# bioinformatics-ua/polus

Measured on AMD Instinct MI355X. Metric: train samples/sec BioBERT-base NER seq256, higher is better.
Workload: dtype bf16; 1 GPU; BERT-base (L=12,H=768,A=12,I=3072,V=28996) token classification C=4, seq_len=256, 64 samples/GPU, AdamW lr 5e-5 wd 0.01 warm-up 10%, dropout 0.1 (hidden + attention) (BASELINE.json configs[2] per-GPU shape), random-init weights; global_batch=64, seq_len=256, parallelism=dp1, grad_allreduce=none

## Files before the change

polus_amd/csrc/common.h:

```cpp
#pragma once
#include <hip/hip_runtime.h>
#include <stdint.h>
#include <stdio.h>
#include <string.h>
#include <math.h>

#include "../../include/polus_hip.h"

typedef __bf16 bf16_t;
typedef __bf16 bf16x8 __attribute__((ext_vector_type(8)));
typedef __bf16 bf16x4 __attribute__((ext_vector_type(4)));
typedef short s16x4 __attribute__((ext_vector_type(4)));
typedef float f32x4 __attribute__((ext_vector_type(4)));

void polus_set_error(const char* fmt, ...);
#define POLUS_FAIL(...) do { polus_set_error(__VA_ARGS__); return POLUS_ERR_INVALID; } while (0)
#define POLUS_REQUIRE(cond, ...) do { if (!(cond)) { polus_set_error(__VA_ARGS__); return POLUS_ERR_INVALID; } } while (0)
#define POLUS_CHECK_LAUNCH(name) do { hipError_t e__ = hipGetLastError(); \
    if (e__ != hipSuccess) { polus_set_error("%s: launch failed: %s", name, hipGetErrorString(e__)); return POLUS_ERR_HIP; } } while (0)
#define POLUS_HIP(call) do { hipError_t e__ = (call); \
    if (e__ != hipSuccess) { polus_set_error("%s failed: %s", #call, hipGetErrorString(e__)); return POLUS_ERR_HIP; } } while (0)

static inline size_t polus_dtype_size(int dt) { return dt == POLUS_BF16 ? 2 : 4; }
static inline bool polus_aligned16(const void* p) { return (((uintptr_t)p) & 15) == 0; }

struct PolusCfg {
    int gemm_pp;
    int gemm_v1;
    int dw_ungrouped;
    int dw_fused_reduce;
    int ln_bwd_blocks;
    int ln_fin_single;
    int gemm_ring128;
    int gemm_auto_split;
    int ln_halfwave;
    int gemm_order;
    int gemm_persist;
    int reserve_cus;
    int attn_bwd_kres;
    int attn_debug;
    int dw_streamk;
    int dw_sk_cus;
    int dw_sk_delta;
    int attn_fused;
};
const PolusCfg& polus_cfg();
int polus_num_cus();
int polus_reserved_cus();

struct PolusDyn { uint32_t salt; float lr, lr_t; uint32_t pad; };
const PolusDyn* polus_dyn();
__device__ __forceinline__ uint32_t polus_eff_seed(uint32_t seed, const PolusDyn* dyn) {
    if (!dyn) return seed;
    uint32_t x = seed + dyn->salt;
    x ^= x >> 15;
    return x * 0x2C1B3C6Du;
}

template <typename T> __device__ __forceinline__ float to_f(T x);
template <> __device__ __forceinline__ float to_f<float>(float x) { return x; }
template <> __device__ __forceinline__ float to_f<bf16_t>(bf16_t x) { return (float)x; }
template <typename T> __device__ __forceinline__ T from_f(float x);
template <> __device__ __forceinline__ float from_f<float>(float x) { return x; }
template <> __device__ __forceinline__ bf16_t from_f<bf16_t>(float x) { return (bf16_t)x; }

template <typename T> __device__ __forceinline__ void load4(const T* p, float (&v)[4]);
template <> __device__ __forceinline__ void load4<float>(const float* p, float (&v)[4]) {
    float4 t = *reinterpret_cast<const float4*>(p); v[0] = t.x; v[1] = t.y; v[2] = t.z; v[3] = t.w;
}
template <> __device__ __forceinline__ void load4<bf16_t>(const bf16_t* p, float (&v)[4]) {
    bf16x4 t = *reinterpret_cast<const bf16x4*>(p);
    v[0] = (float)t[0]; v[1] = (float)t[1]; v[2] = (float)t[2]; v[3] = (float)t[3];
}
template <typename T> __device__ __forceinline__ void store4(T* p, const float (&v)[4]);
template <> __device__ __forceinline__ void store4<float>(float* p, const float (&v)[4]) {
    *reinterpret_cast<float4*>(p) = make_float4(v[0], v[1], v[2], v[3]);
}
template <> __device__ __forceinline__ void store4<bf16_t>(bf16_t* p, const float (&v)[4]) {
    bf16x4 t; t[0] = (bf16_t)v[0]; t[1] = (bf16_t)v[1]; t[2] = (bf16_t)v[2]; t[3] = (bf16_t)v[3];
    *reinterpret_cast<bf16x4*>(p) = t;
}

__device__ __forceinline__ float erf_fast(float x) {
    const float ax = fabsf(x);
    const float t = __frcp_rn(1.0f + 0.3275911f * ax);
    float poly = 1.061405429f;
    poly = poly * t - 1.453152027f;
    poly = poly * t + 1.421413741f;
    poly = poly * t - 0.284496736f;
    poly = poly * t + 0.254829592f;
    const float r = 1.0f - poly * t * __expf(-ax * ax);
    return copysignf(r, x);
}
__device__ __forceinline__ float gelu_f(float x) { return 0.5f * x * (1.0f + erf_fast(x * 0.70710678118654752f)); }
__device__ __forceinline__ float gelu_grad_f(float x) {
    float cdf = 0.5f * (1.0f + erf_fast(x * 0.70710678118654752f));
    float pdf = 0.3989422804014327f * __expf(-0.5f * x * x);
    return cdf + x * pdf;
}
__device__ __forceinline__ float swish_f(float x) { return x / (1.0f + __expf(-x)); }
__device__ __forceinline__ float swish_grad_f(float x) {
    float s = 1.0f / (1.0f + __expf(-x));
    return s * (1.0f + x * (1.0f - s));
}
typedef float f32x2_t __attribute__((ext_vector_type(2)));
__device__ __forceinline__ f32x2_t gelu_poly2(f32x2_t x, const float (&c)[11]) {
    f32x2_t xc = {__builtin_amdgcn_fmed3f(x[0], -4.5f, 4.5f), __builtin_amdgcn_fmed3f(x[1], -4.5f, 4.5f)};
    f32x2_t s = xc * xc;
    f32x2_t u = __builtin_elementwise_fma(s, (f32x2_t){2.0f / 20.25f, 2.0f / 20.25f}, (f32x2_t){-1.0f, -1.0f});
    f32x2_t r = {c[10], c[10]};
#pragma unroll
    for (int k = 9; k >= 0; --k) r = __builtin_elementwise_fma(r, u, (f32x2_t){c[k], c[k]});
    return __builtin_elementwise_fma(xc, r, (f32x2_t){0.5f, 0.5f});
}
__device__ __forceinline__ f32x2_t gelu_cdf2(f32x2_t x) {
    const float q[11] = {1.569049305e-01f, -7.719386095e-02f, 5.470119065e-02f, -4.010921159e-02f, 2.828393083e-02f,
                         -1.902094059e-02f, 1.143922652e-02f, -5.251548121e-03f, 2.716277400e-03f, -2.340015935e-03f,
                         9.806926012e-04f};
    return gelu_poly2(x, q);
}
__device__ __forceinline__ f32x2_t gelu_grad2(f32x2_t x) {
    const float w[11] = {1.594289755e-01f, -9.003904569e-02f, 8.714168751e-02f, -9.350841452e-02f, 9.645831298e-02f,
                         -9.557466143e-02f, 7.437658385e-02f, -3.356380937e-02f, 2.252388123e-02f, -3.068672777e-02f,
                         1.457471506e-02f};
    return gelu_poly2(x, w);
}
// ... 131 lines not shown
```

polus_amd/csrc/norm.hip:

```cpp
#include "common.h"

namespace {

constexpr int MAXC = 8;
constexpr int WAVES = 16;
constexpr int LN_THREADS = 64 * WAVES;
constexpr int MAX_PARTIAL_BLOCKS = 256;

__device__ __forceinline__ int n_chunks(int H) { return (H + 255) >> 8; }

template <typename T, int NC>
__device__ __forceinline__ void load_row(const T* row, int H, int lane, float (&v)[NC][4]) {
#pragma unroll
    for (int c = 0; c < NC; ++c) {
        int col = (lane + 64 * c) * 4;
        if (col < H) load4<T>(row + col, v[c]);
        else { v[c][0] = v[c][1] = v[c][2] = v[c][3] = 0.f; }
    }
}

template <int NC>
__device__ __forceinline__ void load_feat(const float* __restrict__ p, int H, int lane, float (&v)[NC][4]) {
#pragma unroll
    for (int c = 0; c < NC; ++c) {
// ... 170 lines not shown
    }
}

template <typename T, typename TDX, int NC>
__device__ __forceinline__ void ln_bwd_row(const float (&xv)[NC][4], const T* dyrow, const float (&gv)[NC][4],
                                           TDX* dxrow, int H, int lane, float mu, float rs, ColAcc<NC>& acc,
                                           int want_bias, TDX* dxm_row = nullptr, DropArgs out_drop = DropArgs{0, 0, 1.f},
                                           DropArgs in_drop = DropArgs{0, 0, 1.f}, unsigned rowbase = 0) {
    float dy[NC][4];
    load_row<T, NC>(dyrow, H, lane, dy);
    if (in_drop.thresh) {
#pragma unroll
        for (int c = 0; c < NC; ++c) {
            int col = (lane + 64 * c) * 4;
            polus_dropout_run<4>(dy[c], in_drop.seed, rowbase + col, in_drop.thresh, in_drop.inv, true);
        }
    }
    float s1 = 0.f, s2 = 0.f;
    float xh[NC][4], dxh[NC][4];
#pragma unroll
    for (int c = 0; c < NC; ++c) {
        int col = (lane + 64 * c) * 4;
        if (col < H) {
#pragma unroll
            for (int e = 0; e < 4; ++e) {
                xh[c][e] = (xv[c][e] - mu) * rs;
                dxh[c][e] = dy[c][e] * gv[c][e];
                s1 += dxh[c][e];
                s2 += dxh[c][e] * xh[c][e];
                acc.dg[c][e] += dy[c][e] * xh[c][e];
                acc.db[c][e] += dy[c][e];
            }
        } else {
#pragma unroll
            for (int e = 0; e < 4; ++e) xh[c][e] = dxh[c][e] = 0.f;
        }
    }
    s1 = wave_sum(s1) / (float)H;
    s2 = wave_sum(s2) / (float)H;
#pragma unroll
    for (int c = 0; c < NC; ++c) {
        int col = (lane + 64 * c) * 4;
        if (col < H) {
            float o[4], om[4];
#pragma unroll
            for (int e = 0; e < 4; ++e) { o[e] = (dxh[c][e] - s1 - xh[c][e] * s2) * rs; om[e] = o[e]; }
            if (out_drop.thresh) polus_dropout_run<4>(om, out_drop.seed, rowbase + col, out_drop.thresh, out_drop.inv, true);
            if (want_bias) {
#pragma unroll
                for (int e = 0; e < 4; ++e) acc.dbias[c][e] += om[e];
            }
            store4<TDX>(dxrow + col, o);
            if (dxm_row) store4<TDX>(dxm_row + col, om);
        }
    }
}

constexpr int BWD_WAVES = 4, BWD_MAX_BLOCKS = 1024, FIN_GROUP = 128;
template <typename T, int NC>
__global__ __launch_bounds__(64 * BWD_WAVES) void ln_bwd_kernel(const T* __restrict__ dy, const T* __restrict__ x,
                                                     const float* __restrict__ gamma, const float* __restrict__ mean,
                                                     const float* __restrict__ rstd, T* __restrict__ dx,
                                                     float* __restrict__ partial, int rows, int H, int want_bias,
                                                     T* __restrict__ dxm, DropArgs drop) {
    if (drop.thresh) drop.seed = polus_eff_seed(drop.seed, drop.dyn);
    extern __shared__ __attribute__((aligned(16))) unsigned char smem_raw[];
    float* lds = reinterpret_cast<float*>(smem_raw);
    const int lane = threadIdx.x & 63, wid = threadIdx.x >> 6;
    ColAcc<NC> acc;
    colacc_zero(acc);
    float gv[NC][4];
    load_feat<NC>(gamma, H, lane, gv);
    for (int row = blockIdx.x * BWD_WAVES + wid; row < rows; row += gridDim.x * BWD_WAVES) {
        float xv[NC][4];
        load_row<T, NC>(x + (long)row * H, H, lane, xv);
        ln_bwd_row<T, T, NC>(xv, dy + (long)row * H, gv, dx + (long)row * H, H, lane, mean[row], rstd[row], acc, want_bias,
                             dxm ? dxm + (long)row * H : nullptr, drop, DropArgs{0, 0, 1.f}, (unsigned)row * (unsigned)H);
    }
    colacc_flush_par<NC, BWD_WAVES>(acc, lds, partial, H, lane, wid, want_bias);
}

__global__ __launch_bounds__(1024) void colsum_finalize_kernel(const float* __restrict__ partial, int P, int pstride,
                                                               int ncols, int seg, float* out0, float* out1,
                                                               float* out2, int accumulate, int pgroup = 0) {
    __shared__ float red[16][64];
    const int cx = threadIdx.x & 63, gy = threadIdx.x >> 6;
    const int col = blockIdx.x * 64 + cx;
    float s = 0.f;
    if (pgroup > 0) {
        const int p0 = blockIdx.y * pgroup;
        partial += (long)p0 * pstride;
        P = min(pgroup, P - p0);
        out0 += (long)blockIdx.y * ncols;
    }
    if (col < ncols) {
#pragma unroll 8
        for (int p = gy; p < P; p += 16) s += partial[(long)p * pstride + col];
    }
    red[gy][cx] = s;
    __syncthreads();
    if (gy == 0 && col < ncols) {
        float t = 0.f;
#pragma unroll
        for (int k = 0; k < 16; ++k) t += red[k][cx];
        int which = col / seg, c = col % seg;
        float* out = which == 0 ? out0 : which == 1 ? out1 : out2;
        if (out) out[c] = accumulate ? out[c] + t : t;
    }
}

template <int NC>
__global__ __launch_bounds__(64 * BWD_WAVES) void ln_bwd_hw_kernel(const bf16_t* __restrict__ dy, const bf16_t* __restrict__ x,
                                                                    const float* __restrict__ gamma, const float* __restrict__ mean,
                                                                    const float* __restrict__ rstd, bf16_t* __restrict__ dx,
                                                                    float* __restrict__ partial, int rows, int H, int want_bias,
                                                                    bf16_t* __restrict__ dxm, DropArgs drop) {
    if (drop.thresh) drop.seed = polus_eff_seed(drop.seed, drop.dyn);
    extern __shared__ __attribute__((aligned(16))) unsigned char smem_raw[];
    float* lds = reinterpret_cast<float*>(smem_raw);
    const int lane = threadIdx.x & 63, wid = threadIdx.x >> 6, half = lane >> 5, hl = lane & 31;
    float gv[NC][8], adg[NC][8], adb[NC][8], abias[NC][8];
#pragma unroll
    for (int c = 0; c < NC; ++c) {
        const int col = (hl + 32 * c) * 8;
        load4<float>(gamma + col, *reinterpret_cast<float(*)[4]>(&gv[c][0])); load4<float>(gamma + col + 4, *reinterpret_cast<float(*)[4]>(&gv[c][4]));
#pragma unroll
        for (int e = 0; e < 8; ++e) adg[c][e] = adb[c][e] = abias[c][e] = 0.f;
    }
    const float invH = 1.0f / (float)H;
    for (int row = (blockIdx.x * BWD_WAVES + wid) * 2 + half; row < rows; row += gridDim.x * BWD_WAVES * 2) {
        const float mu = mean[row], rs = rstd[row];
        float xh[NC][8], dxh[NC][8];
        float s1 = 0.f, s2 = 0.f;
#pragma unroll
        for (int c = 0; c < NC; ++c) {
            const long off = (long)row * H + (hl + 32 * c) * 8;
            const bf16x8v tx = *reinterpret_cast<const bf16x8v*>(x + off);
            const bf16x8v td = *reinterpret_cast<const bf16x8v*>(dy + off);
#pragma unroll
            for (int e = 0; e < 8; ++e) {
                const float d = (float)td[e];
                xh[c][e] = ((float)tx[e] - mu) * rs;
                dxh[c][e] = d * gv[c][e];
                s1 += dxh[c][e];
                s2 += dxh[c][e] * xh[c][e];
                adg[c][e] += d * xh[c][e];
                adb[c][e] += d;
            }
        }
        s1 = half_sum(s1) * invH;
        s2 = half_sum(s2) * invH;
#pragma unroll
        for (int c = 0; c < NC; ++c) {
            const int col = (hl + 32 * c) * 8;
            float o[8], om[8];
#pragma unroll
            for (int e = 0; e < 8; ++e) { o[e] = (dxh[c][e] - s1 - xh[c][e] * s2) * rs; om[e] = o[e]; }
            if (drop.thresh) polus_dropout_run<8>(om, drop.seed, (unsigned)row * (unsigned)H + col, drop.thresh, drop.inv, true);
            if (want_bias) {
#pragma unroll
                for (int e = 0; e < 8; ++e) abias[c][e] += om[e];
            }
            bf16x8v t;
#pragma unroll
            for (int e = 0; e < 8; ++e) t[e] = (bf16_t)o[e];
            *reinterpret_cast<bf16x8v*>(dx + (long)row * H + col) = t;
            if (dxm) {
#pragma unroll
                for (int e = 0; e < 8; ++e) t[e] = (bf16_t)om[e];
                *reinterpret_cast<bf16x8v*>(dxm + (long)row * H + col) = t;
            }
        }
    }
    float* mine = lds + (long)wid * 3 * H;
#pragma unroll
    for (int c = 0; c < NC; ++c) {
        const int col = (hl + 32 * c) * 8;
#pragma unroll
        for (int e = 0; e < 8; ++e) {
            adg[c][e] += __shfl_xor(adg[c][e], 32, 64);
            adb[c][e] += __shfl_xor(adb[c][e], 32, 64);
            abias[c][e] += __shfl_xor(abias[c][e], 32, 64);
        }
        if (half == 0) {
            *reinterpret_cast<float4*>(mine + col) = make_float4(adg[c][0], adg[c][1], adg[c][2], adg[c][3]);
            *reinterpret_cast<float4*>(mine + col + 4) = make_float4(adg[c][4], adg[c][5], adg[c][6], adg[c][7]);
            *reinterpret_cast<float4*>(mine + H + col) = make_float4(adb[c][0], adb[c][1], adb[c][2], adb[c][3]);
            *reinterpret_cast<float4*>(mine + H + col + 4) = make_float4(adb[c][4], adb[c][5], adb[c][6], adb[c][7]);
            *reinterpret_cast<float4*>(mine + 2 * H + col) = make_float4(abias[c][0], abias[c][1], abias[c][2], abias[c][3]);
// ... 116 lines not shown
    const int rows = B * S;
    float gv[NC][4], bv[NC][4];
    load_feat<NC>(gamma, H, lane, gv);
    load_feat<NC>(beta, H, lane, bv);
    for (int row = blockIdx.x * WAVES + wid; row < rows; row += gridDim.x * WAVES) {
        int id = ids[row]; id = id < 0 ? 0 : (id >= vocab ? vocab - 1 : id);
        int tt = tts ? tts[row] : 0; tt = tt < 0 ? 0 : (tt >= type_vocab ? type_vocab - 1 : tt);
        float v[NC][4];
        gather_sum<T, NC>(word, pos, type, id, row % S, tt, H, lane, v);
        float mu, rs;
        row_stats<NC>(v, H, lane, eps, mu, rs);
        normalize_store<T, NC>(v, gv, bv, y + (long)row * H, H, lane, mu, rs, dthresh, dseed, dinv, (unsigned)row * (unsigned)H);
        if (lane == 0) { mean[row] = mu; rstd[row] = rs; }
    }
}

template <typename T, int NC>
__global__ __launch_bounds__(LN_THREADS) void embed_bwd_ln_kernel(const T* __restrict__ dy, const int32_t* __restrict__ ids,
                                                           const int32_t* __restrict__ tts, const float* __restrict__ word,
                                                           const float* __restrict__ pos, const float* __restrict__ type,
                                                           const float* __restrict__ gamma, const float* __restrict__ mean,
                                                           const float* __restrict__ rstd, float* __restrict__ de,
                                                           float* __restrict__ partial, int B, int S, int H, int vocab,
                                                           int type_vocab, DropArgs in_drop) {
    if (in_drop.thresh) in_drop.seed = polus_eff_seed(in_drop.seed, in_drop.dyn);
    extern __shared__ __attribute__((aligned(16))) unsigned char smem_raw[];
    float* lds = reinterpret_cast<float*>(smem_raw);
    const int lane = threadIdx.x & 63, wid = threadIdx.x >> 6;
    const int rows = B * S;
    ColAcc<NC> acc;
    colacc_zero(acc);
    float gv[NC][4];
    load_feat<NC>(gamma, H, lane, gv);
    for (int row = blockIdx.x * WAVES + wid; row < rows; row += gridDim.x * WAVES) {
        int id = ids[row]; id = id < 0 ? 0 : (id >= vocab ? vocab - 1 : id);
        int tt = tts ? tts[row] : 0; tt = tt < 0 ? 0 : (tt >= type_vocab ? type_vocab - 1 : tt);
        float xv[NC][4];
        gather_sum<T, NC>(word, pos, type, id, row % S, tt, H, lane, xv);
        ln_bwd_row<T, float, NC>(xv, dy + (long)row * H, gv, de + (long)row * H, H, lane, mean[row], rstd[row], acc, 0,
                                 nullptr, DropArgs{0, 0, 1.f}, in_drop, (unsigned)row * (unsigned)H);
    }
    colacc_flush(acc, lds, partial, H, lane, wid, 0);
}

constexpr int SC_RUN = 8, SC_WAVES = 8;
template <int NC>
__global__ __launch_bounds__(64 * SC_WAVES) void embed_scatter_atomic_kernel(const float* __restrict__ de, const int32_t* __restrict__ ids,
                                                                      float* __restrict__ gword, int rows, int H, int vocab) {
    const int lane = threadIdx.x & 63, wid = threadIdx.x >> 6;
    const long stride = (long)gridDim.x * SC_WAVES * SC_RUN;
    for (long r0 = ((long)blockIdx.x * SC_WAVES + wid) * SC_RUN; r0 < rows; r0 += stride) {
        int mine = -1;
        if (lane < SC_RUN && r0 + lane < rows) { mine = ids[r0 + lane]; mine = mine < 0 ? 0 : (mine >= vocab ? vocab - 1 : mine); }
        float row[SC_RUN][NC][4];
#pragma unroll
        for (int j = 0; j < SC_RUN; ++j) {
            const bool valid = r0 + j < rows;
            const float* src = de + (r0 + j) * H + lane;
#pragma unroll
            for (int c = 0; c < NC; ++c)
#pragma unroll
                for (int k = 0; k < 4; ++k)
                    row[j][c][k] = (valid && c * 256 + k * 64 + lane < H) ? src[c * 256 + k * 64] : 0.f;
        }
#pragma unroll
        for (int t = 0; t < SC_RUN; ++t) {
            const int id = __shfl(mine, t, 64);
            const unsigned same = (unsigned)__ballot(mine == id);
            if (id < 0 || (same & ((1u << t) - 1u))) continue;
            float* dst = gword + (long)id * H + lane;
#pragma unroll
            for (int c = 0; c < NC; ++c)
#pragma unroll
                for (int k = 0; k < 4; ++k) {
                    float acc = row[t][c][k];
#pragma unroll
                    for (int j = t + 1; j < SC_RUN; ++j)
                        if ((same >> j) & 1u) acc += row[j][c][k];
                    if (c * 256 + k * 64 + lane < H) atomicAdd(dst + c * 256 + k * 64, acc);
                }
        }
    }
}
__global__ __launch_bounds__(LN_THREADS) void embed_scatter_atomic_wide_kernel(const float* __restrict__ de, const int32_t* __restrict__ ids,
                                                                        float* __restrict__ gword, int rows, int H, int vocab) {
    const int lane = threadIdx.x & 63, wid = threadIdx.x >> 6;
    for (int row = blockIdx.x * WAVES + wid; row < rows; row += gridDim.x * WAVES) {
        int id = ids[row]; id = id < 0 ? 0 : (id >= vocab ? vocab - 1 : id);
        const float* src = de + (long)row * H;
        float* dst = gword + (long)id * H;
        for (int col = lane; col < H; col += 64) atomicAdd(dst + col, src[col]);
    }
}

__global__ __launch_bounds__(LN_THREADS) void embed_scatter_owner_kernel(const float* __restrict__ de, const int32_t* __restrict__ ids,
                                                                  float* __restrict__ gword, int rows, int H, int vocab) {
    const int lane = threadIdx.x & 63, wid = threadIdx.x >> 6;
    for (int row = blockIdx.x * WAVES + wid; row < rows; row += gridDim.x * WAVES) {
        auto clampid = [vocab](int v) { return v < 0 ? 0 : (v >= vocab ? vocab - 1 : v); };
        const int cid = clampid(ids[row]);
        bool dup = false;
        for (int j0 = 0; j0 < row && !dup; j0 += 64) {
            int j = j0 + lane;
            bool hit = (j < row) && (clampid(ids[j]) == cid);
            dup = __any(hit);
        }
        if (dup) continue;
        float* dst = gword + (long)cid * H;
        for (int c0 = 0; c0 < H; c0 += 64 * 4) {
            int col = c0 + lane * 4;
            float a[4] = {0.f, 0.f, 0.f, 0.f};
            for (int j0 = row; j0 < rows; j0 += 64) {
                int j = j0 + lane;
                unsigned long long m = __ballot((j < rows) && (clampid(ids[j]) == cid));
                while (m) {
                    int b = __ffsll((long long)m) - 1;
                    m &= m - 1;
                    if (col < H) {
                        float v[4];
                        load4<float>(de + (long)(j0 + b) * H + col, v);
#pragma unroll
                        for (int e = 0; e < 4; ++e) a[e] += v[e];
                    }
                }
            }
            if (col < H) {
                float o[4];
                load4<float>(dst + col, o);
#pragma unroll
                for (int e = 0; e < 4; ++e) o[e] += a[e];
                store4<float>(dst + col, o);
            }
        }
    }
}

__global__ __launch_bounds__(256) void embed_pos_grad_kernel(const float* __restrict__ de, float* __restrict__ gpos,
                                                             int B, int S, int H, int accumulate) {
    long idx = (long)blockIdx.x * blockDim.x + threadIdx.x;
    if (idx >= (long)S * H) return;
    float s = 0.f;
    for (int b = 0; b < B; ++b) s += de[(long)b * S * H + idx];
    gpos[idx] = accumulate ? gpos[idx] + s : s;
}

}

extern "C" size_t polus_layernorm_bwd_workspace_bytes(int rows, int H) {
    int b = ln_bwd_blocks(rows), b2 = ln_blocks(rows);
    if (b2 > b) b = b2;
    int groups = (b + FIN_GROUP - 1) / FIN_GROUP;
    return ((size_t)b + groups) * 3 * (size_t)H * sizeof(float);
}

extern "C" int polus_layernorm_fwd(int dtype, const void* x, const float* gamma, const float* beta,
                                   void* y, float* mean, float* rstd, int rows, int H, float eps, void* stream) {
    POLUS_REQUIRE(x && gamma && beta && y && mean && rstd, "polus_layernorm_fwd: null pointer");
    POLUS_REQUIRE(rows > 0 && H > 0 && H % 4 == 0 && H <= 256 * MAXC, "polus_layernorm_fwd: H=%d must be a multiple of 4, <= %d", H, 256 * MAXC);
    POLUS_REQUIRE(polus_aligned16(x) && polus_aligned16(y) && polus_aligned16(gamma) && polus_aligned16(beta),
                  "polus_layernorm_fwd: pointers must be 16-byte aligned");
    hipStream_t st = static_cast<hipStream_t>(stream);
    int blocks = (rows + WAVES - 1) / WAVES;
    if (blocks > 4096) blocks = 4096;
    if (dtype == POLUS_BF16 && H % 256 == 0 && H <= 1024 && rows % 2 == 0 && polus_cfg().ln_halfwave) {
        const int fw = 4;
        int hb = (rows / 2 + fw - 1) / fw;
// ... 71 lines not shown
    const int ncols = (dbias ? 3 : 2) * H;
    if (blocks > polus_cfg().ln_fin_single) {
        int groups = (blocks + FIN_GROUP - 1) / FIN_GROUP;
        float* part2 = partial + (size_t)blocks * 3 * H;
        hipLaunchKernelGGL(colsum_finalize_kernel, dim3((ncols + 63) / 64, groups), dim3(1024), 0, st,
                           partial, blocks, 3 * H, ncols, ncols, part2, (float*)nullptr, (float*)nullptr, 0, FIN_GROUP);
        POLUS_CHECK_LAUNCH("polus_layernorm_bwd_finalize(1)");
        hipLaunchKernelGGL(colsum_finalize_kernel, dim3((ncols + 63) / 64), dim3(1024), 0, st,
                           part2, groups, ncols, ncols, H, dgamma, dbeta, dbias, accumulate, 0);
    } else {
        hipLaunchKernelGGL(colsum_finalize_kernel, dim3((ncols + 63) / 64), dim3(1024), 0, st,
                           partial, blocks, 3 * H, ncols, H, dgamma, dbeta, dbias, accumulate, 0);
    }
    POLUS_CHECK_LAUNCH("polus_layernorm_bwd_finalize");
    return POLUS_OK;
}

extern "C" size_t polus_colsum_workspace_bytes(int rows, int cols) {
    int chunks = (rows + 63) / 64;
    if (chunks > 256) chunks = 256;
    if (chunks < 1) chunks = 1;
    return (size_t)chunks * (size_t)cols * sizeof(float);
}

extern "C" int polus_colsum(int dtype, const void* x, long ldx, int rows, int cols, float* out, int accumulate,
                            void* workspace, size_t workspace_bytes, void* stream) {
    POLUS_REQUIRE(x && out && rows > 0 && cols > 0 && ldx >= cols, "polus_colsum: bad arguments");
    POLUS_REQUIRE(dtype == POLUS_F32 || dtype == POLUS_BF16, "polus_colsum: bad dtype");
    return colsum_launch(dtype, x, ldx, rows, cols, out, accumulate, nullptr, 0, workspace, workspace_bytes,
                         static_cast<hipStream_t>(stream));
}

extern "C" size_t polus_embed_bwd_workspace_bytes(int B, int S, int H) {
    size_t rows = (size_t)B * S;
    size_t de = rows * H * sizeof(float);
    size_t part = polus_layernorm_bwd_workspace_bytes((int)rows, H);
    size_t cs = polus_colsum_workspace_bytes((int)rows, H);
    return de + (part > cs ? part : cs) + 256;
}

extern "C" int polus_embed_ln_fwd(int dtype, const int32_t* ids, const int32_t* type_ids,
                                  const float* word, const float* pos, const float* type,
                                  const float* gamma, const float* beta, void* y, float* mean, float* rstd,
                                  int B, int S, int H, int vocab, int max_pos, int type_vocab, float eps,
                                  float drop_p, uint32_t seed, void* stream) {
    POLUS_REQUIRE(ids && word && pos && type && gamma && beta && y && mean && rstd, "polus_embed_ln_fwd: null pointer");
    POLUS_REQUIRE(drop_p >= 0.f && drop_p < 1.f, "polus_embed_ln_fwd: bad drop_p");
    const unsigned dthresh = drop_p > 0.f ? polus_drop_thresh(drop_p) : 0u;
    const float dinv = 1.0f / (1.0f - drop_p);
    POLUS_REQUIRE(B > 0 && S > 0 && S <= max_pos, "polus_embed_ln_fwd: S=%d exceeds max_position_embeddings=%d", S, max_pos);
    POLUS_REQUIRE(H % 4 == 0 && H <= 256 * MAXC && vocab > 0 && type_vocab > 0, "polus_embed_ln_fwd: bad H=%d", H);
    POLUS_REQUIRE(polus_aligned16(word) && polus_aligned16(pos) && polus_aligned16(type) && polus_aligned16(y) &&
                  polus_aligned16(gamma) && polus_aligned16(beta), "polus_embed_ln_fwd: pointers must be 16-byte aligned");
    hipStream_t st = static_cast<hipStream_t>(stream);
    int rows = B * S, blocks = (rows + WAVES - 1) / WAVES;
    if (blocks > 4096) blocks = 4096;
    if (dtype == POLUS_BF16)
        POLUS_NC_DISPATCH(H, bf16_t, embed_fwd_kernel, dim3(blocks), dim3(LN_THREADS), 0, st, ids, type_ids, word, pos, type, gamma, beta, (bf16_t*)y, mean, rstd, B, S, H, vocab, type_vocab, eps, dthresh, seed, dinv, polus_dyn());
    else if (dtype == POLUS_F32)
        POLUS_NC_DISPATCH(H, float, embed_fwd_kernel, dim3(blocks), dim3(LN_THREADS), 0, st, ids, type_ids, word, pos, type, gamma, beta, (float*)y, mean, rstd, B, S, H, vocab, type_vocab, eps, dthresh, seed, dinv, polus_dyn());
    else POLUS_FAIL("polus_embed_ln_fwd: bad dtype");
    POLUS_CHECK_LAUNCH("polus_embed_ln_fwd");
    return POLUS_OK;
}

extern "C" int polus_embed_ln_bwd(int dtype, const void* dy, const int32_t* ids, const int32_t* type_ids,
                                  const float* word, const float* pos, const float* type, const float* gamma,
                                  const float* mean, const float* rstd,
                                  float* gword, float* gpos, float* gtype, float* ggamma, float* gbeta,
                                  int accumulate, int deterministic,
                                  int B, int S, int H, int vocab, int max_pos, int type_vocab,
                                  float drop_p, uint32_t seed,
                                  void* workspace, size_t workspace_bytes, void* stream) {
    DropArgs in_drop{drop_p > 0.f ? polus_drop_thresh(drop_p) : 0u, seed, 1.0f / (1.0f - drop_p), polus_dyn()};
    POLUS_REQUIRE(dy && ids && word && pos && type && gamma && mean && rstd && gword && gpos && gtype && ggamma && gbeta,
                  "polus_embed_ln_bwd: null pointer");
    POLUS_REQUIRE(B > 0 && S > 0 && S <= max_pos && H % 4 == 0 && H <= 256 * MAXC, "polus_embed_ln_bwd: bad shape");
    POLUS_REQUIRE(polus_aligned16(dy) && polus_aligned16(gword) && polus_aligned16(workspace),
                  "polus_embed_ln_bwd: pointers must be 16-byte aligned");
    size_t need = polus_embed_bwd_workspace_bytes(B, S, H);
    if (!workspace || workspace_bytes < need) { polus_set_error("polus_embed_ln_bwd: workspace %zu < %zu", workspace_bytes, need); return POLUS_ERR_WORKSPACE; }
    hipStream_t st = static_cast<hipStream_t>(stream);
    const int rows = B * S;
    float* de = static_cast<float*>(workspace);
    size_t de_bytes = ((size_t)rows * H * sizeof(float) + 255) / 256 * 256;
    float* partial = reinterpret_cast<float*>(static_cast<unsigned char*>(workspace) + de_bytes);
    size_t partial_bytes = workspace_bytes - de_bytes;
    int blocks = ln_blocks(rows);
    size_t lds = 3 * (size_t)H * sizeof(float);
    if (dtype == POLUS_BF16)
        POLUS_NC_DISPATCH(H, bf16_t, embed_bwd_ln_kernel, dim3(blocks), dim3(LN_THREADS), lds, st, (const bf16_t*)dy, ids, type_ids, word, pos, type, gamma, mean, rstd, de, partial, B, S, H, vocab, type_vocab, in_drop);
    else if (dtype == POLUS_F32)
        POLUS_NC_DISPATCH(H, float, embed_bwd_ln_kernel, dim3(blocks), dim3(LN_THREADS), lds, st, (const float*)dy, ids, type_ids, word, pos, type, gamma, mean, rstd, de, partial, B, S, H, vocab, type_vocab, in_drop);
    else POLUS_FAIL("polus_embed_ln_bwd: bad dtype");
    POLUS_CHECK_LAUNCH("polus_embed_ln_bwd(ln)");
    hipLaunchKernelGGL(colsum_finalize_kernel, dim3((2 * H + 63) / 64), dim3(1024), 0, st,
                       partial, blocks, 3 * H, 2 * H, H, ggamma, gbeta, (float*)nullptr, accumulate);
    POLUS_CHECK_LAUNCH("polus_embed_ln_bwd(finalize)");

    if (!accumulate) {
        POLUS_HIP(hipMemsetAsync(gword, 0, (size_t)vocab * H * sizeof(float), st));
        POLUS_HIP(hipMemsetAsync(gpos, 0, (size_t)max_pos * H * sizeof(float), st));
    }
    int sblocks = (rows + WAVES - 1) / WAVES;
    if (sblocks > 4096) sblocks = 4096;
    if (deterministic)
        hipLaunchKernelGGL(embed_scatter_owner_kernel, dim3(sblocks), dim3(LN_THREADS), 0, st, de, ids, gword, rows, H, vocab);
    else
    {
        const dim3 g(min((rows + SC_RUN * SC_WAVES - 1) / (SC_RUN * SC_WAVES), 4096)), b(64 * SC_WAVES);
        if (H <= 256) hipLaunchKernelGGL(embed_scatter_atomic_kernel<1>, g, b, 0, st, de, ids, gword, rows, H, vocab);
        else if (H <= 512) hipLaunchKernelGGL(embed_scatter_atomic_kernel<2>, g, b, 0, st, de, ids, gword, rows, H, vocab);
        else if (H <= 768) hipLaunchKernelGGL(embed_scatter_atomic_kernel<3>, g, b, 0, st, de, ids, gword, rows, H, vocab);
        else if (H <= 1024) hipLaunchKernelGGL(embed_scatter_atomic_kernel<4>, g, b, 0, st, de, ids, gword, rows, H, vocab);
        else hipLaunchKernelGGL(embed_scatter_atomic_wide_kernel, dim3(sblocks), dim3(LN_THREADS), 0, st, de, ids, gword, rows, H, vocab);
    }
    POLUS_CHECK_LAUNCH("polus_embed_ln_bwd(scatter)");
    hipLaunchKernelGGL(embed_pos_grad_kernel, dim3(((long)S * H + 255) / 256), dim3(256), 0, st, de, gpos, B, S, H, accumulate);
    POLUS_CHECK_LAUNCH("polus_embed_ln_bwd(pos)");
    for (int t = 0; t < type_vocab; ++t) {
        if (type_ids) {
            int rc = colsum_launch(POLUS_F32, de, H, rows, H, gtype + (long)t * H, accumulate, type_ids, t, partial, partial_bytes, st);
            if (rc != POLUS_OK) return rc;
        } else if (t == 0) {
            int rc = colsum_launch(POLUS_F32, de, H, rows, H, gtype, accumulate, nullptr, 0, partial, partial_bytes, st);
            if (rc != POLUS_OK) return rc;
        } else if (!accumulate) {
            POLUS_HIP(hipMemsetAsync(gtype + (long)t * H, 0, (size_t)H * sizeof(float), st));
        }
    }
    return POLUS_OK;
}
```

polus_amd/csrc/runtime.hip:

```cpp
#include "common.h"
#include <stdarg.h>

static thread_local char g_err[512] = "";

void polus_set_error(const char* fmt, ...) {
    va_list ap;
    va_start(ap, fmt);
    vsnprintf(g_err, sizeof(g_err), fmt, ap);
    va_end(ap);
}

extern "C" const char* polus_last_error(void) { return g_err; }

static PolusCfg g_cfg;
static bool g_cfg_ready = false;
static int env_int(const char* name, int dflt) {
    const char* e = getenv(name);
    return (e && *e) ? atoi(e) : dflt;
}
static void read_cfg() {
    g_cfg.gemm_pp = env_int("POLUS_GEMM_PP", 0);
    g_cfg.gemm_v1 = getenv("POLUS_GEMM_V1") != nullptr;
    g_cfg.dw_ungrouped = getenv("POLUS_DW_UNGROUPED") != nullptr;
    g_cfg.gemm_order = env_int("POLUS_GEMM_ORDER", 4);
    g_cfg.reserve_cus = env_int("POLUS_GEMM_RESERVE_CUS", 0);
    g_cfg.gemm_persist = env_int("POLUS_GEMM_PERSIST", 1);
    g_cfg.dw_fused_reduce = env_int("POLUS_DW_FUSED_REDUCE", 1);
    g_cfg.attn_fused = env_int("POLUS_ATTN_FUSED", 1);
    g_cfg.attn_bwd_kres = env_int("POLUS_ATTN_BWD_KRES", 1);
    g_cfg.attn_debug = env_int("POLUS_ATTN_DEBUG", 0);
    g_cfg.ln_halfwave = env_int("POLUS_LN_HALFWAVE", 1);
    g_cfg.gemm_auto_split = env_int("POLUS_GEMM_AUTO_SPLIT", 1);
    g_cfg.gemm_ring128 = env_int("POLUS_GEMM_RING128", 0);
    g_cfg.ln_bwd_blocks = env_int("POLUS_LN_BWD_BLOCKS", 512);
    g_cfg.ln_fin_single = env_int("POLUS_LN_FIN_SINGLE", 512);
    g_cfg.dw_streamk = env_int("POLUS_DW_STREAMK", 0);
    g_cfg.dw_sk_delta = env_int("POLUS_DW_SK_DELTA", 2);
    g_cfg.dw_sk_cus = env_int("POLUS_DW_SK_CUS", 0);
    g_cfg_ready = true;
}
const PolusCfg& polus_cfg() {
    if (!g_cfg_ready) read_cfg();
    return g_cfg;
}
extern "C" int polus_reload_env(void) { read_cfg(); return POLUS_OK; }

int polus_num_cus() {
    static int n = 0;
    if (!n) {
        int dev = 0; hipDeviceProp_t prop;
        if (hipGetDevice(&dev) == hipSuccess && hipGetDeviceProperties(&prop, dev) == hipSuccess) n = prop.multiProcessorCount;
        if (n <= 0) n = 256;
    }
    return n;
}
static int g_reserve_on = 1;
extern "C" int polus_set_reserve_active(int on) { g_reserve_on = on != 0; return POLUS_OK; }
int polus_reserved_cus() { return g_reserve_on ? polus_cfg().reserve_cus : 0; }

static const PolusDyn* g_dyn = nullptr;
const PolusDyn* polus_dyn() { return g_dyn; }
extern "C" int polus_set_dynamic_params(const void* dev_block16) {
    POLUS_REQUIRE(dev_block16 == nullptr || polus_aligned16(dev_block16), "polus_set_dynamic_params: the block must be 16-byte aligned");
    g_dyn = static_cast<const PolusDyn*>(dev_block16);
    return POLUS_OK;
}
extern "C" int polus_abi_version(void) { return POLUS_ABI_VERSION; }

extern "C" int polus_device_info(int* n_cu, int* lds_bytes_per_cu, char* arch, int arch_len) {
    int dev = 0;
    POLUS_HIP(hipGetDevice(&dev));
    hipDeviceProp_t prop;
    POLUS_HIP(hipGetDeviceProperties(&prop, dev));
    if (n_cu) *n_cu = prop.multiProcessorCount;
    if (lds_bytes_per_cu) *lds_bytes_per_cu = (int)prop.maxSharedMemoryPerMultiProcessor;
    if (arch && arch_len > 0) {
        strncpy(arch, prop.gcnArchName, arch_len - 1);
        arch[arch_len - 1] = 0;
    }
    return POLUS_OK;
}

namespace {

template <typename S, typename D>
__global__ void cast_kernel(const S* __restrict__ src, D* __restrict__ dst, int64_t n) {
    int64_t i4 = ((int64_t)blockIdx.x * blockDim.x + threadIdx.x) * 4;
    const int64_t stride = (int64_t)gridDim.x * blockDim.x * 4;
    for (; i4 < n; i4 += stride) {
        if (i4 + 4 <= n) {
            float v[4];
            load4<S>(src + i4, v);
            store4<D>(dst + i4, v);
        } else {
            for (int64_t j = i4; j < n; ++j) dst[j] = from_f<D>(to_f<S>(src[j]));
        }
    }
}

__global__ void scale_kernel(float* __restrict__ x, float a, int64_t n) {
    int64_t i4 = ((int64_t)blockIdx.x * blockDim.x + threadIdx.x) * 4;
    const int64_t stride = (int64_t)gridDim.x * blockDim.x * 4;
    for (; i4 < n; i4 += stride) {
        if (i4 + 4 <= n) {
            float4 v = *reinterpret_cast<float4*>(x + i4);
            v.x *= a; v.y *= a; v.z *= a; v.w *= a;
            *reinterpret_cast<float4*>(x + i4) = v;
        } else {
            for (int64_t j = i4; j < n; ++j) x[j] *= a;
        }
    }
}

template <typename T>
__global__ void act_bwd_kernel(const T* __restrict__ dy, const T* __restrict__ u, T* __restrict__ du, int64_t n, int act) {
    int64_t i4 = ((int64_t)blockIdx.x * blockDim.x + threadIdx.x) * 4;
    const int64_t stride = (int64_t)gridDim.x * blockDim.x * 4;
    for (; i4 < n; i4 += stride) {
        if (i4 + 4 <= n) {
            float a[4], b[4];
            load4<T>(dy + i4, a);
// ... 188 lines not shown
```

polus_amd/models.py:

```python
import json
import os
import sys
from functools import wraps

import numpy as np
import torch

from . import _lib, ops
from .layers import CRF, Dense, Dropout, Flatten, Layer, dense_bwd_params_group, gemm_dx
from .tensor import ParamArena, to_device, device
from .utils import complex_json_deserializer, complex_json_serializer, flatten_dict, merge_dicts

COMPUTE_DTYPES = {"f32": torch.float32, "float32": torch.float32, torch.float32: torch.float32,
                  "bf16": torch.bfloat16, "bfloat16": torch.bfloat16, torch.bfloat16: torch.bfloat16}


def load_model(file_name_w_ext, change_config={}, external_module=None):
    file_name = os.path.splitext(file_name_w_ext)[0]
    with open(file_name_w_ext, "r") as f:
        cfg = complex_json_deserializer(json.load(f))
    cfg["model"] = merge_dicts(cfg.get("model", {}), change_config)
    module = external_module if external_module is not None else sys.modules[__name__]
    model = getattr(module, cfg["func_name"])(**cfg)
    if os.path.exists(file_name + ".init.npz"):
# ... 306 lines not shown
        l2 = logits.reshape(-1, logits.shape[-1])
        if l2.dtype != torch.float32:
            l2 = l2.float()
        out = torch.empty(l2.shape[0], dtype=torch.int32, device=l2.device)
        ops.argmax(l2.contiguous(), out)
        return out.view(logits.shape[:-1])


class Sequential(PolusModel):

    def __init__(self, layers, compute_dtype="f32", name=None, input_dim=None):
        super().__init__(name)
        self.layers = list(layers)
        self.compute_dtype = COMPUTE_DTYPES[compute_dtype]
        self.arena = ParamArena(self.compute_dtype)
        feat = input_dim
        for i, l in enumerate(self.layers):
            feat = l.build(self.arena, feat, f"{l.name}{i}")
        last_dense = [l for l in self.layers if isinstance(l, Dense)]
        if last_dense and last_dense[-1].activation is None and last_dense[-1].out_dtype is None:
            last_dense[-1].out_dtype = torch.float32
        self.arena.finalize()

    def call(self, x, training=False, **kw):
        x = to_device(x, None, self.arena.device)
        if x.is_floating_point() and x.dtype != self.compute_dtype:
            x = x.to(self.compute_dtype)
        for l in self.layers:
            x = l.forward(x, training=training)
        return x

    def backward(self, dy, accumulate=False):
        first_param_layer = next(i for i, l in enumerate(self.layers) if l.variables())
        for i in range(len(self.layers) - 1, -1, -1):
            l = self.layers[i]
            if isinstance(l, Dense):
                dy = l.backward(dy, accumulate, need_dx=(i > first_param_layer))
            else:
                dy = l.backward(dy, accumulate)
            self._notify(l.variables())
            if dy is None:
                break
        return dy


class SequentialSavableModel(Sequential, SavableModel):
    pass


class SequentialPolusClassifier(Sequential, PolusClassifier):
    pass


class BertModel(SavableModel):

    def __init__(self, cfg, compute_dtype="bf16", num_labels=None, seed=1234, name="bert", with_embeddings=True,
                 layer_indices=None, arena=None, add_pooling_layer=False):
        super().__init__(name)
        self.config = cfg
        self.compute_dtype = COMPUTE_DTYPES[compute_dtype]
        self.savable_config = {"func_name": "bert_model",
                               "model": dict(cfg.to_dict(), compute_dtype="bf16" if self.compute_dtype == torch.bfloat16 else "f32",
                                             num_labels=num_labels, seed=seed, add_pooling_layer=add_pooling_layer)}
        own = arena is None
        self.arena = arena or ParamArena(self.compute_dtype)
        rng = np.random.Generator(np.random.PCG64(seed))
        self.embeddings = BertEmbeddings(cfg, self.arena, rng) if with_embeddings else None
        idx = range(cfg.num_hidden_layers) if layer_indices is None else layer_indices
        self.layer = [BertLayer(cfg, self.arena, i, rng) for i in idx]
        self.pooler = None
        if add_pooling_layer:
            self.pooler = Dense(cfg.hidden_size, activation="tanh", name="pooler")
            self.pooler.build(self.arena, cfg.hidden_size, "pooler")
        self.head = None
        if num_labels:
            self.head = Dense(num_labels, out_dtype=torch.float32, name="head")
            self.head.build(self.arena, cfg.hidden_size, "head")
        if own:
            self.arena.finalize()
        self._scratch = {}
        self.dropout_base_seed = seed
        self.dropout_step = 0
        self.overlap_dw = os.environ.get("POLUS_OVERLAP_DW", "1") != "0"
        self._side = None

    def scratch(self, key, shape, dtype=None):
        dtype = dtype or self.compute_dtype
        t = self._scratch.get(key)
        if t is None or t.shape != tuple(shape) or t.dtype != dtype:
            t = self._scratch[key] = torch.empty(tuple(shape), dtype=dtype, device=self.arena.device)
        return t

    def load_numpy_params(self, params, head_w=None, head_b=None):
        for v in self.arena.vars:
            if v.name in params:
                v.assign(params[v.name])
        if self.head is not None and head_w is not None:
            self.head.w.assign(head_w)
            self.head.b.assign(head_b)

    def site_seed(self, layer, site, step=None):
        base = self.dropout_base_seed
        if not getattr(self, "identical_dropout_across_ranks", False):
            from . import comm
            if comm.size() > 1:
                base = (base ^ (comm.rank() * 0x9E3779B1)) & 0xFFFFFFFF
        if getattr(self, "graph_seeds", False):
            return dropout_seed_static(base, layer, site)
        return dropout_seed(base, self.dropout_step if step is None else step, layer, site)

    def encode(self, hidden, attention_mask, B, S, training=False):
        cfg = self.config
        p_hid = cfg.hidden_dropout_prob if training else 0.0
        p_att = cfg.attention_probs_dropout_prob if training else 0.0
        for l in self.layer:
            seeds = tuple(self.site_seed(l.index, k) for k in range(3))
            hidden = l.forward(hidden, attention_mask, B, S, p_hid, p_att, seeds, for_backward=training)
        return hidden

    def call(self, input_ids=None, attention_mask=None, token_type_ids=None, training=False, hidden_states=None, **kw):
        dev = self.arena.device
        if isinstance(input_ids, dict):
            d = input_ids
            input_ids, attention_mask = d.get("input_ids"), d.get("attention_mask", attention_mask)
            token_type_ids = d.get("token_type_ids", token_type_ids)
        if attention_mask is not None:
            attention_mask = to_device(attention_mask, torch.int32, dev)
        if hidden_states is None:
            input_ids = to_device(input_ids, torch.int32, dev)
            B, S = input_ids.shape
            if token_type_ids is not None:
                token_type_ids = to_device(token_type_ids, torch.int32, dev)
            hidden = self.embeddings.forward(input_ids, token_type_ids, self.compute_dtype,
                                             self.config.hidden_dropout_prob if training else 0.0, self.site_seed(-1, 0))
        else:
            hs = to_device(hidden_states, self.compute_dtype, dev)
            B, S = hs.shape[0], hs.shape[1]
            hidden = hs.reshape(B * S, -1)
        self._shape = (B, S)
        self.tokens_per_step = B * S
        hidden = self.encode(hidden, attention_mask, B, S, training)
        if training:
            self.dropout_step += 1
        H = self.config.hidden_size
        if self.head is not None:
            return self.head.forward(hidden).view(B, S, -1)
        h3 = hidden.view(B, S, H)
        if self.pooler is not None:
            return BaseModelOutputWithPooling(last_hidden_state=h3, pooler_output=self.pooler.forward(h3[:, 0, :], training))
        return BaseModelOutputWithPooling(last_hidden_state=h3, pooler_output=h3[:, 0, :])

    def backward(self, dy=None, accumulate=False, dpooled=None):
        B, S = self._shape
        H = self.config.hidden_size
        if self.head is not None:
            dy = self.head.backward(dy.reshape(B * S, -1), accumulate)
            self._notify(self.head.variables())
        else:
            if dy is None:
                dy = torch.zeros((B * S, H), dtype=self.compute_dtype, device=self.arena.device)
            else:
                dy = to_device(dy, self.compute_dtype, self.arena.device).reshape(B * S, H)
            if dpooled is not None:
                dy = dy.clone()
                d3 = dy.view(B, S, H)
                dp = to_device(dpooled, self.compute_dtype, self.arena.device).reshape(B, H)
                if self.pooler is not None:
                    dcls = self.pooler.backward(dp, accumulate, dx_resid=d3[:, 0, :])
                    self._notify(self.pooler.variables())
                else:
                    dcls = self.scratch("dcls", (B, H))
                    ops.gemm(dp, _identity(H, self.compute_dtype, self.arena.device), dcls, resid=d3[:, 0, :])
                d3[:, 0, :].copy_(dcls)
        if self.overlap_dw and self._side is None:
            self._side = torch.cuda.Stream(device=self.arena.device)
        side = self._side if self.overlap_dw else None
        pending = []
        main = torch.cuda.current_stream()

        def retire(lay):
            if lay.dw_done is not None:
                main.wait_event(lay.dw_done)
            self._notify(lay.variables())
        for l in reversed(self.layer):
            if len(pending) == 2:
                retire(pending.pop(0))
            dy = l.backward(dy, self.scratch, accumulate, side)
            pending.append(l)
        for lay in pending:
            retire(lay)
        if self.embeddings is not None:
            self.embeddings.backward(dy, accumulate, self.deterministic)
            self._notify(self.embeddings.variables())
            return None
        return dy.view(B, S, -1)

    def inference(self, x):
        logits = self(**x, training=False) if isinstance(x, dict) else self(x, training=False)
        l2 = logits.reshape(-1, logits.shape[-1]).contiguous()
        out = torch.empty(l2.shape[0], dtype=torch.int32, device=l2.device)
        ops.argmax(l2, out)
        return out.view(logits.shape[:-1])


_EYE = {}


def _identity(n, dtype, dev):
    k = (n, dtype, str(dev))
    if k not in _EYE:
        _EYE[k] = torch.eye(n, dtype=dtype, device=dev)
    return _EYE[k]


@from_config
def bert_model(**kw):
    cfg_keys = ("vocab_size", "hidden_size", "num_hidden_layers", "num_attention_heads", "intermediate_size",
                "max_position_embeddings", "type_vocab_size", "layer_norm_eps", "hidden_dropout_prob",
                "attention_probs_dropout_prob", "_name_or_path")
    cfg = BertConfig(**{k: kw[k] for k in cfg_keys if k in kw})
    return BertModel(cfg, compute_dtype=kw.get("compute_dtype", "bf16"), num_labels=kw.get("num_labels"),
                     seed=kw.get("seed", 1234), add_pooling_layer=kw.get("add_pooling_layer", False))


class TFBertSplited(PolusModel):

    def __init__(self, bert_layers, arena, config, run_in_training_mode=True, name="bert_splited"):
        super().__init__(name)
        self.layer = list(bert_layers)
        self.arena, self.config = arena, config
        self.run_in_training_mode = run_in_training_mode
        self.compute_dtype = arena.compute_dtype
        self._scratch = {}
        self.dropout_base_seed, self.dropout_step = 4321, 0

    scratch = BertModel.scratch
    site_seed = BertModel.site_seed

    @property
    def trainable_weights(self):
        return [v for l in self.layer for v in l.variables()]

    def call(self, hidden_states, attention_mask, training=False, **kw):
        dev = self.arena.device
        hs = to_device(hidden_states, self.compute_dtype, dev)
        B, S, H = hs.shape
        mask = to_device(attention_mask, torch.int32, dev)
        hidden = hs.reshape(B * S, H)
        train = bool(self.run_in_training_mode and training)
        p_hid = self.config.hidden_dropout_prob if train else 0.0
        p_att = self.config.attention_probs_dropout_prob if train else 0.0
        for l in self.layer:
            hidden = l.forward(hidden, mask, B, S, p_hid, p_att, tuple(self.site_seed(l.index, k) for k in range(3)), for_backward=bool(training))
        if train:
            self.dropout_step += 1
        self._shape = (B, S)
        self.tokens_per_step = B * S
        h3 = hidden.view(B, S, H)
        return BaseModelOutputWithPooling(last_hidden_state=h3, pooler_output=h3[:, 0, :])

    def backward(self, dy, accumulate=False):
        B, S = self._shape
        dy = to_device(dy, self.compute_dtype, self.arena.device).reshape(B * S, -1)
        for l in reversed(self.layer):
            dy = l.backward(dy, self.scratch, accumulate)
            self._notify(l.variables())
        return dy.view(B, S, -1)


def split_bert_model(bert_model, index_layer, init_models=False, return_pre_bert_model=True,
                     return_post_bert_model=True):
    assert return_pre_bert_model or return_post_bert_model
    L = bert_model.config.num_hidden_layers
    assert L > index_layer > -L and index_layer != 0
    post_model = None
# ... 20 lines not shown
```

Baseline: 5357 samples/s.

## Fuse embedding LayerNorm backward with gradient scatter and reorder embed backward

Adds a fused embedding backward kernel that recomputes the embedding sum, runs the LayerNorm backward, scatters word gradients atomically, and accumulates position and token-type gradients plus gamma/beta partials in one pass. This avoids materialising the full fp32 embedding gradient in workspace and the separate scatter and reduction kernels. The finalize kernel gains a fourth output for the type gradient. Separately, the embedding backward is now issued before waiting on the pending side-stream weight-gradient events, so it can overlap with the last layers' dW work. This costs extra LDS traffic and cross-wave reductions inside the kernel.

```diff
diff --git a/polus_amd/csrc/common.h b/polus_amd/csrc/common.h
--- a/polus_amd/csrc/common.h
+++ b/polus_amd/csrc/common.h
@@ -42,6 +42,7 @@
     int dw_streamk;
     int dw_sk_cus;
     int dw_sk_delta;
+    int embed_fused;
     int attn_fused;
 };
 const PolusCfg& polus_cfg();
diff --git a/polus_amd/csrc/norm.hip b/polus_amd/csrc/norm.hip
--- a/polus_amd/csrc/norm.hip
+++ b/polus_amd/csrc/norm.hip
@@ -276,7 +276,8 @@
 
 __global__ __launch_bounds__(1024) void colsum_finalize_kernel(const float* __restrict__ partial, int P, int pstride,
                                                                int ncols, int seg, float* out0, float* out1,
-                                                               float* out2, int accumulate, int pgroup = 0) {
+                                                               float* out2, int accumulate, int pgroup = 0,
+                                                               float* out3 = nullptr) {
     __shared__ float red[16][64];
     const int cx = threadIdx.x & 63, gy = threadIdx.x >> 6;
     const int col = blockIdx.x * 64 + cx;
@@ -298,7 +299,7 @@
 #pragma unroll
         for (int k = 0; k < 16; ++k) t += red[k][cx];
         int which = col / seg, c = col % seg;
-        float* out = which == 0 ? out0 : which == 1 ? out1 : out2;
+        float* out = which == 0 ? out0 : which == 1 ? out1 : which == 2 ? out2 : out3;
         if (out) out[c] = accumulate ? out[c] + t : t;
     }
 }
@@ -581,6 +582,127 @@
         }
     }
 }
+constexpr int EF_WAVES = 8, EF_MAX_BLOCKS = 1024, EF_RUN4 = 4;
+template <typename T, int NC, int RUN>
+__global__ __launch_bounds__(64 * EF_WAVES) void embed_bwd_fused_kernel(const T* __restrict__ dy, const int32_t* __restrict__ ids,
+                                                                 const int32_t* __restrict__ tts, const float* __restrict__ word,
+                                                                 const float* __restrict__ pos, const float* __restrict__ type,
+                                                                 const float* __restrict__ gamma, const float* __restrict__ mean,
+                                                                 const float* __restrict__ rstd, float* __restrict__ gword,
+                                                                 float* __restrict__ pos_out, long pos_gstride,
+                                                                 float* __restrict__ partial, int B, int S, int H, int vocab,
+                                                                 int type_vocab, DropArgs in_drop) {
+    if (in_drop.thresh) in_drop.seed = polus_eff_seed(in_drop.seed, in_drop.dyn);
+    extern __shared__ __attribute__((aligned(16))) unsigned char smem_raw[];
+    float* lds = reinterpret_cast<float*>(smem_raw);
+    const int lane = threadIdx.x & 63, wid = threadIdx.x >> 6;
+    const int pruns = (S + RUN - 1) / RUN, items = pruns * ((B + EF_WAVES - 1) / EF_WAVES);
+    ColAcc<NC> acc;
+    colacc_zero(acc);
+    float at[2][NC][4];
+#pragma unroll
+    for (int c = 0; c < NC; ++c)
+#pragma unroll
+        for (int e = 0; e < 4; ++e) at[0][c][e] = at[1][c][e] = 0.f;
+    float gv[NC][4];
+    load_feat<NC>(gamma, H, lane, gv);
+    for (int item = blockIdx.x; item < items; item += gridDim.x) {
+        const int bg = item / pruns, s0 = (item - bg * pruns) * RUN;
+        const int b = bg * EF_WAVES + wid;
+        const long r0 = (long)b * S + s0;
+        int mine = -1, mytt = 0;
+        float mymu = 0.f, myrs = 0.f;
+        if (b < B && lane < RUN && s0 + lane < S) {
+            mine = ids[r0 + lane]; mine = mine < 0 ? 0 : (mine >= vocab ? vocab - 1 : mine);
+            if (tts) mytt = tts[r0 + lane];
+            mymu = mean[r0 + lane]; myrs = rstd[r0 + lane];
+        }
+        float row[RUN][NC][4];
+#pragma unroll
+        for (int j = 0; j < RUN; ++j) {
+            float* set = lds + (long)(j & 1) * EF_WAVES * H;
+            float* slice = set + (long)wid * H;
+            const int id = __shfl(mine, j, 64), traw = __shfl(mytt, j, 64);
+            if (id >= 0) {
+                const int tt = traw < 0 ? 0 : (traw >= type_vocab ? type_vocab - 1 : traw);
+                const long r = r0 + j;
+                float xv[NC][4];
+                gather_sum<T, NC>(word, pos, type, id, s0 + j, tt, H, lane, xv);
+                ln_bwd_row<T, float, NC>(xv, dy + r * H, gv, slice, H, lane, __shfl(mymu, j, 64), __shfl(myrs, j, 64), acc, 0,
+                                         nullptr, DropArgs{0, 0, 1.f}, in_drop, (unsigned)r * (unsigned)H);
+                if (traw == 0 || traw == 1) {
+#pragma unroll
+                    for (int c = 0; c < NC; ++c) {
+                        const int col = (lane + 64 * c) * 4;
+                        if (col < H) {
+                            float o[4];
+                            load4<float>(slice + col, o);
+#pragma unroll
+                            for (int e = 0; e < 4; ++e) { if (traw == 0) at[0][c][e] += o[e]; else at[1][c][e] += o[e]; }
+                        }
+                    }
+                }
+            } else {
+                for (int col = lane * 4; col < H; col += 256) *reinterpret_cast<float4*>(slice + col) = make_float4(0.f, 0.f, 0.f, 0.f);
+            }
+            __syncthreads();
+#pragma unroll
+            for (int c = 0; c < NC; ++c)
+#pragma unroll
+                for (int k = 0; k < 4; ++k)
+                    row[j][c][k] = (c * 256 + k * 64 + lane < H) ? slice[c * 256 + k * 64 + lane] : 0.f;
+            if (s0 + j < S) {
+                float* dst = pos_out + bg * pos_gstride + (long)(s0 + j) * H;
+                for (int idx = threadIdx.x; idx < H; idx += 64 * EF_WAVES) {
+                    float t = set[idx];
+#pragma unroll
+                    for (int w = 1; w < EF_WAVES; ++w) t += set[(long)w * H + idx];
+                    dst[idx] = pos_gstride ? t : dst[idx] + t;
+                }
+            }
+        }
+#pragma unroll
+        for (int t = 0; t < RUN; ++t) {
+            const int id = __shfl(mine, t, 64);
+            const unsigned same = (unsigned)__ballot(mine == id);
+            if (id < 0 || (same & ((1u << t) - 1u))) continue;
+            float* dst = gword + (long)id * H + lane;
+#pragma unroll
+            for (int c = 0; c < NC; ++c)
+#pragma unroll
+                for (int k = 0; k < 4; ++k) {
+                    float a = row[t][c][k];
+#pragma unroll
+                    for (int j = t + 1; j < RUN; ++j)
+                        if ((same >> j) & 1u) a += row[j][c][k];
+                    if (c * 256 + k * 64 + lane < H) atomicAdd(dst + c * 256 + k * 64, a);
+                }
+        }
+    }
+    float* dst = partial + (long)blockIdx.x * 4 * H;
+#pragma unroll
+    for (int pass = 0; pass < 2; ++pass) {
+        __syncthreads();
+#pragma unroll
+        for (int c = 0; c < NC; ++c) {
+            const int col = (lane + 64 * c) * 4;
+            if (col < H) {
+                store4<float>(lds + (long)wid * H + col, pass ? at[0][c] : acc.dg[c]);
+                store4<float>(lds + (long)(EF_WAVES + wid) * H + col, pass ? at[1][c] : acc.db[c]);
+            }
+        }
+        __syncthreads();
+        for (int idx = threadIdx.x; idx < 2 * H; idx += 64 * EF_WAVES) {
+            const int v = idx >= H;
+            const float* src = lds + (long)v * EF_WAVES * H + (idx - v * H);
+            float t = src[0];
+#pragma unroll
+            for (int w = 1; w < EF_WAVES; ++w) t += src[(long)w * H];
+            dst[pass * 2 * H + idx] = t;
+        }
+    }
+}
+
 __global__ __launch_bounds__(LN_THREADS) void embed_scatter_atomic_wide_kernel(const float* __restrict__ de, const int32_t* __restrict__ ids,
                                                                         float* __restrict__ gword, int rows, int H, int vocab) {
     const int lane = threadIdx.x & 63, wid = threadIdx.x >> 6;
@@ -818,6 +940,39 @@
     if (!workspace || workspace_bytes < need) { polus_set_error("polus_embed_ln_bwd: workspace %zu < %zu", workspace_bytes, need); return POLUS_ERR_WORKSPACE; }
     hipStream_t st = static_cast<hipStream_t>(stream);
     const int rows = B * S;
+    if (polus_cfg().embed_fused && !deterministic && H <= 1024 && type_vocab <= 2 && (dtype == POLUS_BF16 || dtype == POLUS_F32)) {
+        const int run = H <= 768 ? SC_RUN : EF_RUN4;
+        const int bgroups = (B + EF_WAVES - 1) / EF_WAVES, items = bgroups * ((S + run - 1) / run);
+        const int blocks = items < EF_MAX_BLOCKS ? items : EF_MAX_BLOCKS;
+        const size_t part_bytes = ((size_t)blocks * 4 * H * sizeof(float) + 255) / 256 * 256;
+        const size_t pos_bytes = bgroups > 1 ? (size_t)bgroups * S * H * sizeof(float) : 0;
+        if (part_bytes + pos_bytes <= workspace_bytes) {
+            float* partial = static_cast<float*>(workspace);
+            float* pos_part = reinterpret_cast<float*>(static_cast<unsigned char*>(workspace) + part_bytes);
+            if (!accumulate) {
+                POLUS_HIP(hipMemsetAsync(gword, 0, (size_t)vocab * H * sizeof(float), st));
+                POLUS_HIP(hipMemsetAsync(gpos, 0, (size_t)max_pos * H * sizeof(float), st));
+            }
+            float* pos_out = bgroups > 1 ? pos_part : gpos;
+            const long pos_gstride = bgroups > 1 ? (long)S * H : 0;
+            const size_t lds = 2 * (size_t)EF_WAVES * H * sizeof(float);
+#define POLUS_EMBED_FUSED(TT, NCV, RUNV) hipLaunchKernelGGL((embed_bwd_fused_kernel<TT, NCV, RUNV>), dim3(blocks), dim3(64 * EF_WAVES), lds, st, (const TT*)dy, ids, type_ids, word, pos, type, gamma, mean, rstd, gword, pos_out, pos_gstride, partial, B, S, H, vocab, type_vocab, in_drop)
+#define POLUS_EMBED_FUSED_NC(TT) do { if (H <= 256) POLUS_EMBED_FUSED(TT, 1, SC_RUN); else if (H <= 512) POLUS_EMBED_FUSED(TT, 2, SC_RUN); else if (H <= 768) POLUS_EMBED_FUSED(TT, 3, SC_RUN); else POLUS_EMBED_FUSED(TT, 4, EF_RUN4); } while (0)
+            if (dtype == POLUS_BF16) POLUS_EMBED_FUSED_NC(bf16_t); else POLUS_EMBED_FUSED_NC(float);
+#undef POLUS_EMBED_FUSED_NC
+#undef POLUS_EMBED_FUSED
+            POLUS_CHECK_LAUNCH("polus_embed_ln_bwd(fused)");
+            const int ncols = (type_vocab == 2 && (type_ids || !accumulate) ? 4 : 3) * H;
+            hipLaunchKernelGGL(colsum_finalize_kernel, dim3((ncols + 63) / 64), dim3(1024), 0, st,
+                               partial, blocks, 4 * H, ncols, H, ggamma, gbeta, gtype, accumulate, 0, gtype + H);
+            POLUS_CHECK_LAUNCH("polus_embed_ln_bwd(fused finalize)");
+            if (bgroups > 1) {
+                hipLaunchKernelGGL(embed_pos_grad_kernel, dim3(((long)S * H + 255) / 256), dim3(256), 0, st, pos_part, gpos, bgroups, S, H, 1);
+                POLUS_CHECK_LAUNCH("polus_embed_ln_bwd(fused pos)");
+            }
+            return POLUS_OK;
+        }
+    }
     float* de = static_cast<float*>(workspace);
     size_t de_bytes = ((size_t)rows * H * sizeof(float) + 255) / 256 * 256;
     float* partial = reinterpret_cast<float*>(static_cast<unsigned char*>(workspace) + de_bytes);
diff --git a/polus_amd/csrc/runtime.hip b/polus_amd/csrc/runtime.hip
--- a/polus_amd/csrc/runtime.hip
+++ b/polus_amd/csrc/runtime.hip
@@ -37,6 +37,7 @@
     g_cfg.dw_streamk = env_int("POLUS_DW_STREAMK", 0);
     g_cfg.dw_sk_delta = env_int("POLUS_DW_SK_DELTA", 2);
     g_cfg.dw_sk_cus = env_int("POLUS_DW_SK_CUS", 0);
+    g_cfg.embed_fused = env_int("POLUS_EMBED_FUSED", 1);
     g_cfg_ready = true;
 }
 const PolusCfg& polus_cfg() {
diff --git a/polus_amd/models.py b/polus_amd/models.py
--- a/polus_amd/models.py
+++ b/polus_amd/models.py
@@ -412,6 +412,7 @@
         self.dropout_base_seed = seed
         self.dropout_step = 0
         self.overlap_dw = os.environ.get("POLUS_OVERLAP_DW", "1") != "0"
+        self.embed_early = os.environ.get("POLUS_EMBED_EARLY", "1") != "0"
         self._side = None
 
     def scratch(self, key, shape, dtype=None):
@@ -517,10 +518,14 @@
                 retire(pending.pop(0))
             dy = l.backward(dy, self.scratch, accumulate, side)
             pending.append(l)
+        early = side is not None and self.embed_early and self.embeddings is not None
+        if early:
+            self.embeddings.backward(dy, accumulate, self.deterministic)
         for lay in pending:
             retire(lay)
         if self.embeddings is not None:
-            self.embeddings.backward(dy, accumulate, self.deterministic)
+            if not early:
+                self.embeddings.backward(dy, accumulate, self.deterministic)
             self._notify(self.embeddings.variables())
             return None
         return dy.view(B, S, -1)
```

Result: no change. 5387 samples/s (median of 6 runs) (+0.6%).
